# WangYuTum/odometry

Hardware: AMD Instinct MI355X
Metric: tracked frames/sec (1241x376, 4-level pyramid) (higher is better)
Workload: dtype f32

## Files before the change

### odometry_amd/csrc/kernels.hip.h

```cpp
#pragma once
#include <hip/hip_runtime.h>
#include "odo_math.h"

#ifndef ODO_PHASE_STAMPS
#define ODO_PHASE_STAMPS 0
#endif
#if ODO_PHASE_STAMPS
#define ODO_DBG(a) ((a).dbg)
#else
#define ODO_DBG(a) ((unsigned long long*)nullptr)
#endif

#ifndef ODO_KERNEL
#define ODO_KERNEL __global__
#define ODO_KERNEL_T __global__
#endif
#ifdef ODO_LM_CHAIN_TU
#define ODO_DEVICE_VAR static __device__
#else
#define ODO_DEVICE_VAR __device__
#endif

namespace odo {

// ... 915 lines not shown
  int n_levels;
  const LmState* st_in;
  LmState* st_out;
  const double* part_in;
  double* part_out;
  float lambda0, precision;
  int robust;
  float huber_delta;
  LmTraceRow* trace;
  float* cost_stat;
  int* host_prog;
  int seq;
  int first_of_solve;
  float init[16];
  unsigned long long* dbg;
  float* out;
  int* done_flag;
  int token;
  LmState* st2[2];
  double* part2[2];
  int min_level;
  int fine_lo;
  unsigned long long* xbuf;
  unsigned fine_dispatch;
  unsigned fine_epoch;
  unsigned fine_wait;
  int fine_home;
  float* chain_pose;
  int* chain_guard;
  int chain_in_token;
  int chain_out;
  float kf_rule[7];
  int stop_level;
  LmState* final_state;
  unsigned long long* span;
  unsigned long long* arm;
};
struct StepLaunch {
  const LmState* st_in; LmState* st_out;
  const double* part_in; double* part_out;
  int seq, first_of_solve;
  unsigned long long* span;
};
static_assert(offsetof(StepArgs, lv) == 0, "lm_copy_levels reads the level table at offset 0 of the StepArgs");
__device__ __forceinline__ const unsigned* lm_kernarg_words() { return (const unsigned*)__builtin_amdgcn_kernarg_segment_ptr(); }
__device__ __forceinline__ void lm_copy_levels(StepLevel* lv_sh, const unsigned* __restrict__ src) {
  constexpr int kWords = (int)(sizeof(StepLevel) * ODO_MAX_LEVELS_K / sizeof(unsigned));
  for (int i = (int)threadIdx.x; i < kWords; i += (int)blockDim.x) ((unsigned*)lv_sh)[i] = src[i];
}
__device__ __forceinline__ bool lm_span_block() {
  return threadIdx.x == 0 && (gridDim.y == 1 || ((blockIdx.x ^ blockIdx.y) & 7u) == 0u);
}
__device__ __forceinline__ void lm_span_begin(unsigned long long* span) {
  if (span && lm_span_block()) atomicMin(span, (unsigned long long)wall_clock64());
}
__device__ __forceinline__ void lm_span_end(unsigned long long* span) {
  if (span && lm_span_block()) atomicMax(span + 1, (unsigned long long)wall_clock64());
}

constexpr int kFoldChunk = 20;

__device__ __forceinline__ void lm_state_machine(bool pending, const StepLevel* lv, int n_levels, float lambda0,
                                                 float precision, LmState& s_sh, double* acc_sh, LmTraceRow* __restrict__ trace,
                                                 float* __restrict__ cost_stat, bool publisher,
                                                 unsigned long long* smdbg = nullptr, int stop_level = 0) {
  const int t = threadIdx.x;
  if (t < 64) {
    unsigned long long c0 = smdbg ? __builtin_readcyclecounter() : 0, c1 = c0, c2 = c0, c3 = c0;
    LmState s = s_sh;
    const int iter0 = s.iter, lvl0 = s.level;
    const float err_last0 = s.err_last;
    bool need_step = false;
    if (pending) need_step = lm_decide(&s, acc_sh, precision);
    if (smdbg) { c1 = __builtin_readcyclecounter(); c2 = c1; c3 = c1; }
    if (need_step) {
      float d[6];
      solve_damped_wave_regs(acc_sh, s.lambda, d);
#pragma unroll
      for (int i = 0; i < 6; i++) s.delta[i] = d[i];
      if (smdbg) { asm volatile("" ::"v"(d[0]), "v"(d[5])); c2 = __builtin_readcyclecounter(); }
#ifdef ODO_NO_LANE_SINCOS
      lm_apply_step(&s, s.max_iters);
#else
      lm_apply_step_wave(&s, s.max_iters);
#endif
      if (smdbg) { asm volatile("" ::"v"(s.T[0]), "v"(s.T[14])); c3 = __builtin_readcyclecounter(); }
    }
    if (smdbg && t == 0) { smdbg[0] += c1 - c0; smdbg[1] += c2 - c1; smdbg[2] += c3 - c2; smdbg[3] += 1; }
    if (pending) {
      if (publisher && t == 0 && trace) {
        const int ev = s.n_evals - 1;
        if (ev < kTraceCap) {
          LmTraceRow& r = trace[ev];
          r.level = lvl0;
          r.iter = iter0;
          r.n_res = (int)acc_sh[28];
          r.err = s.err_now;
          r.accepted = (s.status == 0 && !(s.err_now > err_last0)) ? 1 : 0;
          r.stop = (s.stop_reason == 3 || s.active) ? 0 : s.stop_reason;
          r.lambda_after = s.lambda;
#pragma unroll
          for (int i = 0; i < 6; i++) r.delta[i] = (s.active || s.stop_reason == 3) ? s.delta[i] : 0.0f;
        }
        int evals_this_level = 0;
#pragma unroll
        for (int i = 0; i < 8; i++) evals_this_level += (i == (lvl0 & 7)) ? s.iters_level[i] : 0;
        if (iter0 == 0 && evals_this_level == 1) cost_stat[lvl0 * 2 + 0] = s.err_now;
        cost_stat[lvl0 * 2 + 1] = s.err_now;
      }
      s.pending = 0;
    }
    if (lv) {
      while (!s.active && s.status == 0 && !s.finished) {
        const int next = (s.level < 0) ? n_levels - 1 : s.level - 1;
        if (next < stop_level) { s.finished = 1; break; }
        s.stop_reason = 0;
        lm_begin_level(&s, next, lambda0, lv[next].max_iters);
      }
      if (s.status != 0) s.finished = 1;
    }
    if (t == 0) s_sh = s;
  }
  __syncthreads();
}

struct LmHot {
  Se3 cur, inc;
  float Tc[12];
  float lambda, err_last;
  int level, iter, max_iters, active, status, finished, n_evals, stop_reason;
};
__device__ __forceinline__ void lm_hot_load(LmHot& h, const LmState& s) {
  h.cur = s.cur; h.inc = s.inc;
  float M[16];
  se3_to_colmajor(s.cur, M);
#pragma unroll
  for (int c = 0; c < 4; c++)
#pragma unroll
    for (int r = 0; r < 3; r++) h.Tc[c * 3 + r] = M[c * 4 + r];
  h.lambda = s.lambda; h.err_last = s.err_last;
  h.level = s.level; h.iter = s.iter; h.max_iters = s.max_iters; h.active = s.active; h.status = s.status; h.finished = s.finished;
  h.n_evals = s.n_evals; h.stop_reason = s.stop_reason;
}
__device__ __forceinline__ void lm_hot_store(const LmHot& h, LmState& s) {
  s.cur = h.cur; s.inc = h.inc; s.last = h.cur;
  s.lambda = h.lambda; s.err_last = h.err_last;
  s.level = h.level; s.iter = h.iter; s.max_iters = h.max_iters; s.active = h.active; s.status = h.status; s.finished = h.finished;
  s.n_evals = h.n_evals; s.stop_reason = h.stop_reason;
  s.pending = 0;
}
__device__ __forceinline__ void lm_state_machine_hot(LmHot& h, const StepLevel* lv, int n_levels, float lambda0, float precision,
                                                     LmState& s_sh, const double* acc_sh, LmTraceRow* __restrict__ trace,
                                                     float* __restrict__ cost_stat, bool publisher,
                                                     unsigned long long* smdbg = nullptr, int stop_level = 0) {
  const int t = threadIdx.x;
  if (t < 64) {
    unsigned long long c0 = smdbg ? __builtin_readcyclecounter() : 0, c1 = c0, c2 = c0, c3 = c0;
    const int iter0 = h.iter, lvl0 = h.level;
    const float err_last0 = h.err_last;
    float Tprev[12];
#pragma unroll
    for (int c = 0; c < 4; c++)
#pragma unroll
      for (int r = 0; r < 3; r++) Tprev[c * 3 + r] = s_sh.T[c * 4 + r];
    h.n_evals++;
    if (t == 0) s_sh.iters_level[lvl0 & 7] += 1;
    bool need_step = false;
    float err_now = 0.0f;
    bool have_err = false;
    if (!(acc_sh[28] > 0.0)) {
      h.status = -1;
      h.active = 0;
    } else {
      err_now = (float)(acc_sh[27] / acc_sh[28]);
      have_err = true;
      if (err_now > h.err_last) {
        h.lambda = h.lambda * 5.0f;
        if (h.lambda > 1e+5f) { h.active = 0; h.stop_reason = 2; }
        else need_step = true;
      } else {
        h.cur = h.inc;
#pragma unroll
        for (int i = 0; i < 12; i++) h.Tc[i] = Tprev[i];
        const float err_diff = err_now / h.err_last;
        if (err_diff > precision) { h.active = 0; h.stop_reason = 1; }
        else {
          h.err_last = err_now;
          h.lambda = fmaxf(h.lambda / 5.0f, 1e-5f);
          need_step = true;
        }
      }
    }
    if (smdbg) { c1 = __builtin_readcyclecounter(); c2 = c1; c3 = c1; }
    float d[6] = {0.0f, 0.0f, 0.0f, 0.0f, 0.0f, 0.0f};
    bool new_T = false;
    float Tn[16];
#pragma unroll
    for (int i = 0; i < 16; i++) Tn[i] = 0.0f;
    if (need_step) {
      solve_damped_wave_regs(acc_sh, h.lambda, d);
      if (smdbg) { asm volatile("" ::"v"(d[0]), "v"(d[5])); c2 = __builtin_readcyclecounter(); }
      Se3 dd;
      se3_exp_wave(d, &dd);
      const float C[16] = {h.Tc[0], h.Tc[1], h.Tc[2], 0.0f, h.Tc[3], h.Tc[4], h.Tc[5], 0.0f,
                           h.Tc[6], h.Tc[7], h.Tc[8], 0.0f, h.Tc[9], h.Tc[10], h.Tc[11], 1.0f};
      se3_left_update_mat(dd, C, &h.inc);
      se3_to_colmajor(h.inc, Tn);
      new_T = true;
      h.iter++;
      if (!(h.max_iters > h.iter)) { h.active = 0; h.stop_reason = 3; }
      if (smdbg) { asm volatile("" ::"v"(Tn[0]), "v"(Tn[14])); c3 = __builtin_readcyclecounter(); }
    }
    if (smdbg && t == 0) { smdbg[0] += c1 - c0; smdbg[1] += c2 - c1; smdbg[2] += c3 - c2; smdbg[3] += 1; }
    if (t == 0) {
      if (have_err) s_sh.err_now = err_now;
      if (need_step) {
#pragma unroll
        for (int i = 0; i < 6; i++) s_sh.delta[i] = d[i];
      }
    }
    if (publisher && t == 0 && trace) {
      const int ev = h.n_evals - 1;
      const float e = s_sh.err_now;
      if (ev < kTraceCap) {
        LmTraceRow& r = trace[ev];
        r.level = lvl0;
        r.iter = iter0;
        r.n_res = (int)acc_sh[28];
        r.err = e;
        r.accepted = (h.status == 0 && !(e > err_last0)) ? 1 : 0;
        r.stop = (h.stop_reason == 3 || h.active) ? 0 : h.stop_reason;
        r.lambda_after = h.lambda;
#pragma unroll
        for (int i = 0; i < 6; i++) r.delta[i] = (h.active || h.stop_reason == 3) ? d[i] : 0.0f;
      }
      const int evals_this_level = s_sh.iters_level[lvl0 & 7];
      if (iter0 == 0 && evals_this_level == 1) cost_stat[lvl0 * 2 + 0] = e;
      cost_stat[lvl0 * 2 + 1] = e;
    }
    if (lv) {
      while (!h.active && h.status == 0 && !h.finished) {
        const int next = (h.level < 0) ? n_levels - 1 : h.level - 1;
        if (next < stop_level) { h.finished = 1; break; }
        h.stop_reason = 0;
        h.level = next;
        h.iter = 0;
        h.err_last = 1e+10f;
        h.lambda = lambda0;
        h.inc = h.cur;
        h.max_iters = lv[next].max_iters;
        h.active = (h.status == 0 && h.max_iters > 0) ? 1 : 0;
#pragma unroll
        for (int c = 0; c < 4; c++) {
#pragma unroll
          for (int r = 0; r < 3; r++) Tn[c * 4 + r] = h.Tc[c * 3 + r];
          Tn[c * 4 + 3] = (c == 3) ? 1.0f : 0.0f;
        }
        new_T = true;
      }
      if (h.status != 0) h.finished = 1;
    }
    if (t == 0) {
      if (new_T) {
#pragma unroll
        for (int i = 0; i < 16; i++) s_sh.T[i] = Tn[i];
      }
      s_sh.level = h.level; s_sh.active = h.active; s_sh.status = h.status; s_sh.finished = h.finished;
    }
  }
  __syncthreads();
}

constexpr int kUpdThreads = 1024;
#define ODO_STAMP(i) do { if (STAMP && threadIdx.x == 0) stamps[i] = __builtin_readcyclecounter(); } while (0)
template <bool STAMP>
__device__ __forceinline__ void lm_update_body(LmState* __restrict__ st, const double* __restrict__ partials,
                                               int nblk, int expect_level, float precision, int max_iters,
                                               LmTraceRow* __restrict__ trace, float* __restrict__ cost_stat,
                                               int* __restrict__ host_prog, int seq,
                                               unsigned long long* __restrict__ stamps) {
  ODO_STAMP(0);
  if (!(st->active != 0 && st->level == expect_level)) {
    if (host_prog && threadIdx.x == 0) __hip_atomic_store(host_prog, seq, __ATOMIC_RELAXED, __HIP_MEMORY_SCOPE_SYSTEM);
    return;
  }
  __shared__ double sh[32][32];
  __shared__ double acc_sh[32];
  __shared__ LmState s_sh;
  const int t = threadIdx.x;
  const int q = t & 31, seg = t >> 5;
  double v = 0.0;
  if (q < ODO_NACC) {
    double v0 = 0.0, v1 = 0.0, v2 = 0.0, v3 = 0.0;
    int b = seg;
    for (; b + 96 < nblk; b += 128) {
      v0 += partials[(size_t)b * ODO_NACC + q];
      v1 += partials[(size_t)(b + 32) * ODO_NACC + q];
      v2 += partials[(size_t)(b + 64) * ODO_NACC + q];
      v3 += partials[(size_t)(b + 96) * ODO_NACC + q];
    }
    for (; b < nblk; b += 32) v0 += partials[(size_t)b * ODO_NACC + q];
    v = (v0 + v1) + (v2 + v3);
  }
  ODO_STAMP(1);
  sh[seg][q] = v;
  if (t < (int)(sizeof(LmState) / sizeof(int))) ((int*)&s_sh)[t] = ((const int*)st)[t];
  __syncthreads();
  if (t < ODO_NACC) {
    double a = 0.0;
// ... 465 lines not shown
}
static __global__ void __launch_bounds__(kCoarseBlock) lm_coarse_armed_kernel(StepArgs a, int min_level) {
  const StepLaunch q = {a.st_in, a.st_out, a.part_in, a.part_out, a.seq, a.first_of_solve, a.span};
  lm_coarse_body<false, true>(a, q, min_level, lm_kernarg_words());
}
static __global__ void __launch_bounds__(kCoarseBlock) lm_coarse_full_kernel(StepArgs a, int min_level) {
  const StepLaunch q = {a.st_in, a.st_out, a.part_in, a.part_out, a.seq, a.first_of_solve, a.span};
  lm_coarse_body<true>(a, q, min_level, lm_kernarg_words());
}
#endif
template <bool kFull>
__device__ __forceinline__ void lm_coarse_batch_entry(const StepArgs* __restrict__ table, int seq, int first_of_solve, unsigned long long* span) {
  const StepArgs& a = table[blockIdx.y];
  const StepLaunch q = {a.st2[seq & 1], a.st2[(seq + 1) & 1], a.part2[seq & 1], a.part2[(seq + 1) & 1], seq, first_of_solve, span};
  lm_coarse_body<kFull>(a, q, a.min_level, (const unsigned*)&table[blockIdx.y]);
}
ODO_KERNEL void __launch_bounds__(kCoarseBlock) lm_coarse_kernel_batch(const StepArgs* __restrict__ table, int seq, int first_of_solve,
                                                                       unsigned long long* span) {
  lm_coarse_batch_entry<false>(table, seq, first_of_solve, span);
}
ODO_KERNEL void __launch_bounds__(kCoarseBlock) lm_coarse_full_kernel_batch(const StepArgs* __restrict__ table, int seq, int first_of_solve,
                                                                            unsigned long long* span) {
  lm_coarse_batch_entry<true>(table, seq, first_of_solve, span);
}

constexpr int kFineGran = 2 * ODO_NACC;
constexpr int kFineRowsMax = 160;
constexpr int kFineChunk = 8;
constexpr unsigned kFineWaitTicks = 400000u;
struct FineDeadline {
  unsigned long long t0, c0;
  unsigned limit;
  static __device__ __forceinline__ FineDeadline begin(unsigned limit_ticks) {
    return FineDeadline{(unsigned long long)wall_clock64(), (unsigned long long)__builtin_readcyclecounter(), limit_ticks};
  }
  __device__ __forceinline__ bool expired(int spin) const {
    if ((spin & 31) != 31) return false;
    const unsigned long long dt = (unsigned long long)wall_clock64() - t0;
    if (dt <= (unsigned long long)limit) return false;
    if (dt > 4ull * (unsigned long long)limit) return true;
    return (unsigned long long)__builtin_readcyclecounter() - c0 > 24ull * (unsigned long long)limit;
  }
};
constexpr int kTsThreads = 512, kTsPerThread = 32, kTsMaxWg = 128;
constexpr int kTsXbufWords = 2 * kTsMaxWg * 4;
ODO_KERNEL void __launch_bounds__(kTsThreads) lm_tdist_scale_multi_kernel(const float* __restrict__ res, int n,
                                                                          const LmState* __restrict__ st, int expect_level,
                                                                          float* __restrict__ scale_sqr_out,
                                                                          unsigned long long* __restrict__ xbuf, unsigned epoch,
                                                                          unsigned wait_ticks, int* __restrict__ gave_up, int fault) {
  if (!(st->active != 0 && st->level == expect_level)) return;
  const int G = gridDim.x, g = blockIdx.x, t = threadIdx.x, lane = t & 63, wv = t >> 6;
  const size_t stride = (size_t)G * kTsThreads;
  float e2[kTsPerThread];
  int cnt = 0;
#pragma unroll
  for (int k = 0; k < kTsPerThread; k++) {
    const size_t i = (size_t)g * kTsThreads + t + (size_t)k * stride;
    const float r = (i < (size_t)n) ? res[i] : __builtin_nanf("");
    const bool ok = (r == r);
    e2[k] = ok ? r * r : -1.0f;
    cnt += ok ? 1 : 0;
  }
  __shared__ double wsum[kTsThreads / 64];
  __shared__ double wcnt[kTsThreads / 64];
  __shared__ float sh_sigma;
  __shared__ int sh_done, sh_bail;
  const unsigned wait_limit = wait_ticks ? wait_ticks : 400000u;
  float cur = 5.0f;
  double n_valid = 0.0;
  for (int pass = 0; pass < kTdistMaxPasses; pass++) {
    const float sigma_sqr = cur * cur;
    double s = 0.0;
#pragma unroll
    for (int k = 0; k < kTsPerThread; k++)
      if (e2[k] >= 0.0f) s += (double)tdist_term(e2[k], sigma_sqr);
    const double ws = wave_sum64(s);
    if (pass == 0) {
      const double wc = wave_sum64((double)cnt);
      if (lane == 0) wcnt[wv] = wc;
    }
    if (lane == 0) wsum[wv] = ws;
    __syncthreads();
    if (t < 64) {
      double P = 0.0, C = 0.0;
#pragma unroll
      for (int w = 0; w < kTsThreads / 64; w++) { P += wsum[w]; if (pass == 0) C += wcnt[w]; }
      const unsigned tag = (epoch << 10) | (unsigned)(pass + 1);
      unsigned long long* mine = xbuf + ((size_t)(pass & 1) * kTsMaxWg + g) * 4;
      if (lane == 0 && !(fault && g == 1)) {
        const unsigned long long bits = (unsigned long long)__double_as_longlong(P);
        __hip_atomic_store(mine + 0, ((bits >> 32) << 32) | tag, __ATOMIC_RELAXED, __HIP_MEMORY_SCOPE_AGENT);
        __hip_atomic_store(mine + 1, ((bits & 0xffffffffull) << 32) | tag, __ATOMIC_RELAXED, __HIP_MEMORY_SCOPE_AGENT);
        __hip_atomic_store(mine + 2, ((unsigned long long)(unsigned)(int)C << 32) | tag, __ATOMIC_RELAXED, __HIP_MEMORY_SCOPE_AGENT);
      }
      double a = 0.0, c = 0.0;
      bool all = true;
      const FineDeadline dl = FineDeadline::begin(wait_limit);
      for (int gg = lane; gg < G; gg += 64) {
        const unsigned long long* theirs = xbuf + ((size_t)(pass & 1) * kTsMaxWg + gg) * 4;
        unsigned long long w0 = 0, w1 = 0, w2 = 0;
        bool got = false;
        for (int spin = 0; !got; spin++) {
          w0 = __hip_atomic_load(theirs + 0, __ATOMIC_RELAXED, __HIP_MEMORY_SCOPE_AGENT);
          w1 = __hip_atomic_load(theirs + 1, __ATOMIC_RELAXED, __HIP_MEMORY_SCOPE_AGENT);
          w2 = __hip_atomic_load(theirs + 2, __ATOMIC_RELAXED, __HIP_MEMORY_SCOPE_AGENT);
          got = ((unsigned)w0 == tag) && ((unsigned)w1 == tag) && ((unsigned)w2 == tag);
          if (!got && dl.expired(spin)) break;
        }
        all = all && got;
        a += __longlong_as_double((long long)(((w0 >> 32) << 32) | (w1 >> 32)));
        c += (double)(int)(unsigned)(w2 >> 32);
      }
      const bool everyone = __all(all);
      const double total = wave_sum64(a);
      if (pass == 0) n_valid = wave_sum64(c);
      const float nxt = (n_valid > 0.0) ? tdist_next_sigma(total, (int)n_valid) : cur;
      const bool done = !(n_valid > 0.0) || tdist_converged(nxt, cur);
      if (lane == 0) { sh_sigma = nxt; sh_done = done ? 1 : 0; sh_bail = everyone ? 0 : 1; }
    }
    __syncthreads();
    if (sh_bail) {
      if (t == 0) __hip_atomic_store(gave_up, 1, __ATOMIC_RELAXED, __HIP_MEMORY_SCOPE_AGENT);
      return;
    }
    cur = sh_sigma;
    if (sh_done) break;
  }
  if (g == 0 && t == 0) *scale_sqr_out = cur * cur;
}

constexpr int kFineThreads = 2 * kLmBlock;
constexpr int kFineKMax = 32;
constexpr int kScaleChunks = 4 * 2 * kFineKMax;
constexpr int kScaleWords = 2 * kScaleChunks * 2 + kScaleChunks;
constexpr int kFineScaleOff = 2 * kFineRowsMax * kFineGran + kFineKMax;
static_assert(kFineScaleOff % 2 == 0, "scale granule pairs must be 16-byte aligned");
constexpr int kFineXbufWords = kFineScaleOff + kScaleWords;
constexpr int kTdistMaxEvals = 1023;
typedef unsigned FineG2 __attribute__((ext_vector_type(4)));
typedef __attribute__((address_space(1))) FineG2 FineG2Global;
__device__ __forceinline__ void fine_publish(unsigned long long* __restrict__ buf, int vb, int q, double acc, unsigned tag, bool local) {
  const unsigned long long bits = (unsigned long long)__double_as_longlong(acc);
  unsigned long long* g = buf + (size_t)vb * kFineGran + 2 * q;
  const unsigned long long g0 = ((bits >> 32) << 32) | tag, g1 = (bits << 32) | tag;
  if (local) {
    g[0] = g0;
    g[1] = g1;
  } else {
    __hip_atomic_store(g, g0, __ATOMIC_RELAXED, __HIP_MEMORY_SCOPE_AGENT);
    __hip_atomic_store(g + 1, g1, __ATOMIC_RELAXED, __HIP_MEMORY_SCOPE_AGENT);
  }
}
__device__ __forceinline__ int fine_xcc_id() {
  int v;
  asm volatile("s_getreg_b32 %0, hwreg(HW_REG_XCC_ID)" : "=s"(v));
  return v & 0xf;
}
__device__ __forceinline__ bool fine_on_home(int home) {
  return home >= 0 ? fine_xcc_id() == home : (blockIdx.x & 7u) == 0u;
}
ODO_KERNEL void xcc_probe_kernel(int* __restrict__ out) {
  if (threadIdx.x == 0) out[blockIdx.x] = fine_xcc_id();
}
struct XccIds { int id[8]; };
__device__ __forceinline__ float fine_tdist_sigma(unsigned long long* __restrict__ sbuf, int chunk, int nchunk, unsigned tag_ev,
                                                          float e2, bool valid, bool local, unsigned wait_limit, int* bail,
                                                          double (*td_ws)[8], int* td_cnt) {
  const int lane = threadIdx.x & 63, wv = threadIdx.x >> 6;
  const int vb = chunk >> 2, nvb = nchunk >> 2;
  unsigned long long* cnts = sbuf + 2 * kScaleChunks * 2;
  const int my_cnt = __popcll(__ballot(valid));
  float sigma = 5.0f;
  int n_total = 0;
  for (int pass = 0; pass < kTdistMaxPasses; pass++) {
    const unsigned tag = tag_ev | (unsigned)(pass + 1);
    const double ws = wave_sum64(valid ? (double)tdist_term(e2, sigma * sigma) : 0.0);
    if (lane == 0) { td_ws[pass & 1][wv] = ws; if (pass == 0) td_cnt[wv] = my_cnt; }
    __syncthreads();
    unsigned long long* sums = sbuf + (size_t)(pass & 1) * kScaleChunks * 2;
    if ((wv & 3) == 0 && lane == 0) {
      const double G = ((td_ws[pass & 1][wv] + td_ws[pass & 1][wv + 1]) + td_ws[pass & 1][wv + 2]) + td_ws[pass & 1][wv + 3];
      const int C = td_cnt[wv] + td_cnt[wv + 1] + td_cnt[wv + 2] + td_cnt[wv + 3];
      const unsigned long long bits = (unsigned long long)__double_as_longlong(G);
      const unsigned long long g0 = ((bits >> 32) << 32) | tag, g1 = (bits << 32) | tag;
      const unsigned long long gc = ((unsigned long long)(unsigned)C << 32) | tag;
      if (local) {
        sums[2 * vb] = g0; sums[2 * vb + 1] = g1;
        if (pass == 0) cnts[vb] = gc;
      } else {
        __hip_atomic_store(sums + 2 * vb, g0, __ATOMIC_RELAXED, __HIP_MEMORY_SCOPE_AGENT);
        __hip_atomic_store(sums + 2 * vb + 1, g1, __ATOMIC_RELAXED, __HIP_MEMORY_SCOPE_AGENT);
        if (pass == 0) __hip_atomic_store(cnts + vb, gc, __ATOMIC_RELAXED, __HIP_MEMORY_SCOPE_AGENT);
      }
    }
    FineG2 g = {0, 0, 0, 0};
    unsigned long long gc = 0;
    bool all = false;
    FineDeadline dl = {0ull, 0ull, wait_limit};
    __builtin_amdgcn_s_setprio(0);
    for (int spin = 0; !all; spin++) {
      if (spin == 1) dl = FineDeadline::begin(wait_limit);
      if (spin > 0) { if (dl.expired(spin)) break; __builtin_amdgcn_s_sleep(1); }
      bool mine = true;
      if (lane < nvb) {
        g = *(const volatile FineG2Global*)(sums + 2 * lane);
        if (pass == 0) gc = __hip_atomic_load(cnts + lane, __ATOMIC_RELAXED, __HIP_MEMORY_SCOPE_AGENT);
        mine = (g.x == tag) && (g.z == tag) && (pass != 0 || (unsigned)gc == tag);
      }
      all = __all(mine);
    }
    __builtin_amdgcn_s_setprio(3);
    if (!all) { if (lane == 0) *bail = 1; break; }
    double part = 0.0, cnt = 0.0;
    if (lane < nvb) {
      part = __longlong_as_double((long long)(((unsigned long long)g.y << 32) | (unsigned long long)g.w));
      if (pass == 0) cnt = (double)(unsigned)(gc >> 32);
    }
    const double total = wave_sum64(part);
    if (pass == 0) n_total = (int)wave_sum64(cnt);
    const float nxt = (n_total > 0) ? tdist_next_sigma(total, n_total) : sigma;
    const bool done = (n_total == 0) || tdist_converged(nxt, sigma);
    sigma = nxt;
    if (done) break;
  }
  return sigma;
}
template <bool kTdist, bool kTrace>
__device__ __forceinline__ void lm_fine_body(const StepArgs& a, const StepLaunch& q, int K, int w, unsigned long long* __restrict__ xbuf,
                                             int fault, int lo_level, const unsigned* __restrict__ lv_src) {
#if ODO_PHASE_STAMPS
  const unsigned long long w_entry = (unsigned long long)wall_clock64();
#endif
  __builtin_amdgcn_s_setprio(3);
  const int t = threadIdx.x, tl = t & (kLmBlock - 1), half = t >> 8;
  const bool publisher = (w == 0);
  if (publisher && t == 0 && q.span) atomicMin(q.span, (unsigned long long)wall_clock64());
  __shared__ LmState s_sh;
  __shared__ double fold_sh[8 * 32];
  __shared__ double acc_sh[32];
  __shared__ StepLevel lv_sh[ODO_MAX_LEVELS_K];
  __shared__ float rows_sh2[2][kRowFloats * RowBuf<kLmBlock>::W];
  __shared__ int bail_sh, local_sh;
  __shared__ unsigned long long sm_sh[4];
  float* rows_sh = rows_sh2[half];
  const unsigned tag_base = a.fine_epoch << 8;
  unsigned long long* place = xbuf + 2 * kFineRowsMax * kFineGran;
  const unsigned wait_limit = a.fine_wait ? a.fine_wait : kFineWaitTicks;
  lm_copy_levels(lv_sh, lv_src);
  if (t == 0) {
    bail_sh = 0;
    local_sh = 0;
#pragma unroll
    for (int i = 0; i < 4; i++) sm_sh[i] = 0;
    __hip_atomic_store(place + w, ((unsigned long long)(unsigned)fine_xcc_id() << 32) | tag_base, __ATOMIC_RELAXED, __HIP_MEMORY_SCOPE_AGENT);
  }
  __syncthreads();
  lm_fused_prologue(q.st_in, q.part_in, lv_sh, a.n_levels, a.lambda0, a.precision, s_sh, fold_sh, acc_sh, (kTrace ? a.trace : (LmTraceRow*)nullptr), a.cost_stat,
                    publisher, q.first_of_solve ? a.init : nullptr, a.stop_level, a.chain_in_token ? a.chain_pose : nullptr);
  LmHot hot;
  lm_hot_load(hot, s_sh);
  if (t < 64) {
    bool same = true, got = false;
    if (t < K) {
      unsigned long long pw = 0;
      const FineDeadline dl = FineDeadline::begin(wait_limit);
      for (int spin = 0; !got; spin++) {
        pw = __hip_atomic_load(place + t, __ATOMIC_RELAXED, __HIP_MEMORY_SCOPE_AGENT);
        got = ((unsigned)pw == tag_base);
        if (!got && dl.expired(spin)) break;
      }
      same = got && ((int)(pw >> 32) == fine_xcc_id());
    } else {
      got = true;
    }
    const bool all_got = __all(got), all_same = __all(same);
    if (t == 0) { local_sh = (all_got && all_same) ? 1 : 0; if (!all_got) bail_sh = 1; }
  }
  __syncthreads();
  const bool local = local_sh != 0;
  constexpr int kS = 8;
  const int my_q = tl / kS, my_s = tl % kS;
  int rowA = 0, rowB = 0;
  if (my_q < ODO_NACC) rows_of_quantity(my_q, &rowA, &rowB);
  const int fq = t & 31, fseg = t >> 5;
  PointK pt;
  bool pt_ok = false;
  int pt_level = -1;
  unsigned long long c_eval = 0, c_xchg = 0, c_sm = 0, c_it = 0, c_last = ODO_DBG(a) ? __builtin_readcyclecounter() : 0;
#if ODO_PHASE_STAMPS
  unsigned long long c_first = 0, n_first = 0;
#endif
  const unsigned long long c_begin = c_last, w_begin = ODO_DBG(a) ? (unsigned long long)wall_clock64() : 0;
  auto lap = [&](unsigned long long& sum) {
    if (ODO_DBG(a)) { const unsigned long long now = __builtin_readcyclecounter(); sum += now - c_last; c_last = now; }
  };
  for (int ev = 0; ev < 4096; ev++) {
    const bool run = (s_sh.active != 0 && s_sh.status == 0 && !s_sh.finished && !bail_sh && s_sh.level >= lo_level);
    if (!run) break;
    c_it++;
    const StepLevel& L = lv_sh[s_sh.level];
    const float* I2u = lm_uniform_ptr(L.I2);
    const int nblk = L.nblk;
    const unsigned tag = tag_base + 1u + (unsigned)(ev % 255);
    unsigned long long* buf = xbuf + (size_t)(ev & 1) * kFineRowsMax * kFineGran;
    float T[16];
#pragma unroll
    for (int i = 0; i < 16; i++) T[i] = s_sh.T[i];
#if ODO_PHASE_STAMPS
    const bool first_of_level = (s_sh.level != pt_level);
#endif
    const bool resident = (nblk <= 2 * K) && (L.n <= nblk * kLmBlock);
    if (resident) {
      const int vb = w + half * K;
      if (s_sh.level != pt_level) {
        pt_level = s_sh.level;
        const int idx = vb * kLmBlock + tl;
        pt_ok = vb < nblk && idx < L.n;
        if (pt_ok) pt = load_point(L.pl, idx);
      }
      float r = 0.0f, wgt = 0.0f, J[6] = {0.0f, 0.0f, 0.0f, 0.0f, 0.0f, 0.0f};
      bool valid = false;
      if (pt_ok && point_residual_g<kTdist || kTrace>(pt, T, L.k, I2u, L.rows, L.cols, &r, J)) {
        wgt = robust_weight(r, (kTdist || kTrace) ? a.robust : (a.robust == 1 ? 1 : 0), a.huber_delta, 1.0f);
        valid = true;
      }
      if (kTdist && w < nblk) {
        __shared__ double td_ws_sh[2][8];
        __shared__ int td_cnt_sh[8];
        const float sg = fine_tdist_sigma(xbuf + kFineScaleOff, vb * 4 + (tl >> 6), 4 * nblk,
                                          ((a.fine_epoch & 0xfffu) << 20) | (((unsigned)ev & 0x3ffu) << 10), r * r, valid, local, wait_limit, &bail_sh,
                                          td_ws_sh, td_cnt_sh);
        if (valid) wgt = robust_weight(r, 2, a.huber_delta, sg * sg);
      }
      rows_store_z(rows_sh, RowBuf<kLmBlock>::W, tl, J, wgt, r, valid);
      __syncthreads();
      if (bail_sh) break;
      if (vb < nblk) {
        double accq = 0.0;
        if (my_q < ODO_NACC) accq = rows_accumulate<kLmBlock, kS>(rows_sh, rowA, rowB, my_s, accq);
        accq = rows_butterfly8(accq);
        if (my_q < ODO_NACC && my_s == 0 && !(fault && vb == 0)) fine_publish(buf, vb, my_q, accq, tag, local);
      }
    } else {
      const int rounds = (L.n + nblk * kLmBlock - 1) / (nblk * kLmBlock);
      for (int vb0 = w; vb0 < nblk; vb0 += 2 * K) {
        const int vb = vb0 + half * K;
        double accq = 0.0;
        for (int rd = 0; rd < rounds; rd++) {
          const int idx = (vb + rd * nblk) * kLmBlock + tl;
          float r = 0.0f, wgt = 0.0f, J[6] = {0.0f, 0.0f, 0.0f, 0.0f, 0.0f, 0.0f};
          bool valid = false;
          if (vb < nblk && idx < L.n) {
            const PointK p = load_point(L.pl, idx);
            if (point_residual_g<kTdist || kTrace>(p, T, L.k, I2u, L.rows, L.cols, &r, J)) {
              wgt = robust_weight(r, (kTdist || kTrace) ? a.robust : (a.robust == 1 ? 1 : 0), a.huber_delta, 1.0f);
              valid = true;
            }
          }
          __syncthreads();
          rows_store_z(rows_sh, RowBuf<kLmBlock>::W, tl, J, wgt, r, valid);
          __syncthreads();
          if (my_q < ODO_NACC) accq = rows_accumulate<kLmBlock, kS>(rows_sh, rowA, rowB, my_s, accq);
        }
        accq = rows_butterfly8(accq);
        if (vb < nblk && my_q < ODO_NACC && my_s == 0 && !(fault && vb == 0)) fine_publish(buf, vb, my_q, accq, tag, local);
      }
    }
#if ODO_PHASE_STAMPS
    { const unsigned long long before = c_eval; lap(c_eval); if (first_of_level) { c_first += c_eval - before; n_first++; } }
#else
    lap(c_eval);
#endif
    double v = 0.0;
    __builtin_amdgcn_s_setprio(0);
    if (fq < ODO_NACC && fseg < 8) {
      for (int b0 = fseg; b0 < nblk; b0 += 8 * kFineChunk) {
        FineG2 g2[kFineChunk];
        bool all = false;
        FineDeadline dl = {0ull, 0ull, wait_limit};
        for (int spin = 0; !all; spin++) {
          if (spin == 1) dl = FineDeadline::begin(wait_limit);
          if (spin > 0) { if (dl.expired(spin)) break; __builtin_amdgcn_s_sleep(1); }
          all = true;
#pragma unroll
          for (int u = 0; u < kFineChunk; u++) {
            const int b = b0 + 8 * u;
            if (b < nblk) g2[u] = *(const volatile FineG2Global*)(buf + (size_t)b * kFineGran + 2 * fq);
          }
#pragma unroll
          for (int u = 0; u < kFineChunk; u++) {
            const int b = b0 + 8 * u;
            if (b < nblk) all = all && (g2[u].x == tag) && (g2[u].z == tag);
          }
        }
        if (!all) bail_sh = 1;
#pragma unroll
        for (int u = 0; u < kFineChunk; u++) {
          const int b = b0 + 8 * u;
          if (b < nblk) v += __longlong_as_double((long long)(((unsigned long long)g2[u].y << 32) | (unsigned long long)g2[u].w));
        }
      }
    }
    __builtin_amdgcn_s_setprio(3);
    if (fseg < 8) fold_sh[fseg * 32 + fq] = v;
    __syncthreads();
    if (t < ODO_NACC) {
      double acc = 0.0;
#pragma unroll
      for (int g = 0; g < 8; g++) acc += fold_sh[g * 32 + t];
      acc_sh[t] = acc;
    }
    lap(c_xchg);
    if (bail_sh) break;
    lm_state_machine_hot(hot, lv_sh, a.n_levels, a.lambda0, a.precision, s_sh, acc_sh, (kTrace ? a.trace : (LmTraceRow*)nullptr), a.cost_stat, publisher,
                         (ODO_DBG(a) && publisher) ? sm_sh : nullptr, a.stop_level);
    lap(c_sm);
  }
#if ODO_PHASE_STAMPS
  const unsigned long long w_loop_end = (unsigned long long)wall_clock64();
#endif
  if (t == 0) lm_hot_store(hot, s_sh);
  if (bail_sh && t == 0) { s_sh.status = -2; s_sh.active = 0; s_sh.finished = 1; }
  __syncthreads();
  if (publisher) {
    lm_fused_publish(s_sh, q.st_out, a.host_prog, q.seq, a.token, a.cost_stat, a.out, a.done_flag, a.final_state, chain_out_of(a));
#if ODO_PHASE_STAMPS
    const unsigned long long w_published = (unsigned long long)wall_clock64();
#endif
    if (ODO_DBG(a) && t == 0) { ODO_DBG(a)[128] += c_eval; ODO_DBG(a)[129] += c_xchg; ODO_DBG(a)[130] += c_sm; ODO_DBG(a)[131] += c_it; ODO_DBG(a)[132] += 1; ODO_DBG(a)[133] += local ? 1 : 0;
      ODO_DBG(a)[134] += __builtin_readcyclecounter() - c_begin; ODO_DBG(a)[135] += (unsigned long long)wall_clock64() - w_begin;
#pragma unroll
      for (int i = 0; i < 4; i++) ODO_DBG(a)[136 + i] += sm_sh[i]; }
    if (t == 0 && q.span) atomicMax(q.span + 1, (unsigned long long)wall_clock64());
#if ODO_PHASE_STAMPS
    if (ODO_DBG(a) && t == 0) {
      const unsigned long long now = w_published;
      g_lm_diag[2] = w_loop_end;
      g_lm_diag[19] += c_first; g_lm_diag[20] += n_first;
      g_lm_diag[9] += w_begin - w_entry; g_lm_diag[10] += w_loop_end - w_begin; g_lm_diag[11] += now - w_loop_end;
      if (g_lm_diag[0] && w_entry > g_lm_diag[0] && w_entry - g_lm_diag[0] < 100000ull) { g_lm_diag[12] += w_entry - g_lm_diag[0]; g_lm_diag[15] += 1; }
      g_lm_diag[1] = now; g_lm_diag[13] += 1;
    }
#endif
  }
}
ODO_DEVICE_VAR unsigned g_lm_fine_dispatch[2];
__device__ __forceinline__ bool lm_fine_mid_dispatch() {
  return __hip_atomic_load(&g_lm_fine_dispatch[0], __ATOMIC_RELAXED, __HIP_MEMORY_SCOPE_AGENT) !=
         __hip_atomic_load(&g_lm_fine_dispatch[1], __ATOMIC_RELAXED, __HIP_MEMORY_SCOPE_AGENT);
}
template <bool kTdist, bool kTrace>
__device__ __forceinline__ void lm_fine_entry(const StepArgs& a, int K, unsigned long long* __restrict__ xbuf, int fault, int lo_level,
                                              unsigned* dispatch_words) {
  if (threadIdx.x == 0) {
    if (blockIdx.x == 0) __hip_atomic_store(&dispatch_words[0], a.fine_dispatch, __ATOMIC_RELAXED, __HIP_MEMORY_SCOPE_AGENT);
    if (blockIdx.x == gridDim.x - 1) __hip_atomic_store(&dispatch_words[1], a.fine_dispatch, __ATOMIC_RELAXED, __HIP_MEMORY_SCOPE_AGENT);
  }
  if (!fine_on_home(a.fine_home) || lm_chain_skip(a)) return;
  const StepLaunch q = {a.st_in, a.st_out, a.part_in, a.part_out, a.seq, a.first_of_solve, a.span};
  lm_fine_body<kTdist, kTrace>(a, q, K, (int)(blockIdx.x >> 3), xbuf, fault, lo_level, lm_kernarg_words());
}
#ifdef ODO_LM_CHAIN_TU
static __global__ void __launch_bounds__(kFineThreads) lm_fine_kernel(StepArgs a, int K, unsigned long long* __restrict__ xbuf, int fault,
                                                               int lo_level, unsigned* dispatch_words) {
  lm_fine_entry<false, false>(a, K, xbuf, fault, lo_level, dispatch_words);
}
static __global__ void __launch_bounds__(kFineThreads) lm_fine_trace_kernel(StepArgs a, int K, unsigned long long* __restrict__ xbuf, int fault,
                                                                     int lo_level, unsigned* dispatch_words) {
  lm_fine_entry<false, true>(a, K, xbuf, fault, lo_level, dispatch_words);
}
static __global__ void __launch_bounds__(kFineThreads) lm_fine_tdist_kernel(StepArgs a, int K, unsigned long long* __restrict__ xbuf, int fault,
                                                                     int lo_level, unsigned* dispatch_words) {
  lm_fine_entry<true, true>(a, K, xbuf, fault, lo_level, dispatch_words);
}
#endif
template <bool kTrace>
__device__ __forceinline__ void lm_fine_batch_entry(const StepArgs* __restrict__ table, int n, int K, int seq, int first_of_solve,
                                                    unsigned long long* span, int fault, const XccIds& xcc, unsigned* dispatch_words) {
  int r = (int)(blockIdx.x & 7u);
  if (xcc.id[0] >= 0) {
    const int mine = fine_xcc_id();
#pragma unroll
    for (int c = 0; c < 8; c++) if (xcc.id[c] == mine) r = c;
  }
  if (threadIdx.x == 0 && n > 0) {
    if (blockIdx.x == 0) __hip_atomic_store(&dispatch_words[0], table[0].fine_dispatch, __ATOMIC_RELAXED, __HIP_MEMORY_SCOPE_AGENT);
    if (blockIdx.x == gridDim.x - 1) __hip_atomic_store(&dispatch_words[1], table[0].fine_dispatch, __ATOMIC_RELAXED, __HIP_MEMORY_SCOPE_AGENT);
  }
  const int wa = (int)(blockIdx.x >> 3);
  const int i = (wa / K) * 8 + r, w = wa % K;
  if (i >= n) return;
  const StepArgs& a = table[i];
  const StepLaunch q = {a.st2[seq & 1], a.st2[(seq + 1) & 1], a.part2[seq & 1], a.part2[(seq + 1) & 1], seq, first_of_solve,
                        (i == 0) ? span : nullptr};
  if (a.fine_lo >= a.min_level) {
    if (w == 0) lm_fine_body<false, kTrace>(a, q, 1, 0, a.xbuf, 0, ODO_MAX_LEVELS_K + 1, (const unsigned*)&table[i]);
    return;
  }
  lm_fine_body<false, kTrace>(a, q, K, w, a.xbuf, fault, a.fine_lo, (const unsigned*)&table[i]);
}
ODO_KERNEL void __launch_bounds__(kFineThreads) lm_fine_kernel_batch(const StepArgs* __restrict__ table, int n, int K, int seq,
                                                                     int first_of_solve, unsigned long long* span, int fault, XccIds xcc,
                                                                     unsigned* dispatch_words) {
  lm_fine_batch_entry<false>(table, n, K, seq, first_of_solve, span, fault, xcc, dispatch_words);
}
ODO_KERNEL void __launch_bounds__(kFineThreads) lm_fine_trace_kernel_batch(const StepArgs* __restrict__ table, int n, int K, int seq,
                                                                           int first_of_solve, unsigned long long* span, int fault, XccIds xcc,
                                                                     unsigned* dispatch_words) {
  lm_fine_batch_entry<true>(table, n, K, seq, first_of_solve, span, fault, xcc, dispatch_words);
}

struct FinalizeArgs {
  const LmState* st_in;
  const double* part_in;
  float precision;
  LmTraceRow* trace;
  float* cost_stat;
  LmState* st_out;
  float* out;
  int* done_flag;
  int token;
  int first_of_solve;
  float init[16];
};
ODO_KERNEL void __launch_bounds__(kLmBlock) lm_fused_finalize_kernel(FinalizeArgs a) {
  __shared__ LmState s_sh;
  __shared__ double fold_sh[8 * 32];
  __shared__ double acc_sh[32];
  lm_fused_prologue(a.st_in, a.part_in, nullptr, 0, 0.0f, a.precision, s_sh, fold_sh, acc_sh, a.trace,
                    a.cost_stat, true, a.first_of_solve ? a.init : nullptr);
  if (threadIdx.x < (int)(sizeof(LmState) / sizeof(int))) ((int*)a.st_out)[threadIdx.x] = ((const int*)&s_sh)[threadIdx.x];
  if (threadIdx.x == 0) lm_write_result(s_sh, a.cost_stat, a.out, a.done_flag, a.token);
}

ODO_KERNEL void solve_damped_wave_test_kernel(const double* __restrict__ acc_in, float lambda, float* __restrict__ out) {
  __shared__ double acc_sh[32];
  __shared__ float delta_sh[6];
  if (threadIdx.x < ODO_NACC) acc_sh[threadIdx.x] = acc_in[threadIdx.x];
  __syncthreads();
  solve_damped_wave(acc_sh, lambda, delta_sh);
  __syncthreads();
  if (threadIdx.x < 6) out[threadIdx.x] = delta_sh[threadIdx.x];
}

ODO_KERNEL void lm_begin_solve_kernel(LmState* __restrict__ st, const float* __restrict__ init, float* __restrict__ cost_stat) {
  if (threadIdx.x == 0) {
    LmState s;
    float m[16];
    for (int i = 0; i < 16; i++) m[i] = init[i];
    lm_begin_solve(&s, m);
    s.level = -1; s.iter = 0; s.lambda = 0.0f; s.err_last = 1e+10f;
    for (int i = 0; i < 16; i++) s.T[i] = m[i];
    *st = s;
    for (int i = 0; i < 16; i++) cost_stat[i] = 0.0f;
  }
}

ODO_KERNEL void lm_begin_level_kernel(LmState* __restrict__ st, int level, float lambda0, int max_iters) {
  if (threadIdx.x == 0) {
    LmState s = *st;
    s.stop_reason = 0;
    lm_begin_level(&s, level, lambda0, max_iters);
    *st = s;
  }
}

__device__ __forceinline__ void lm_finalize_body(const LmState* __restrict__ st, float* __restrict__ out);
ODO_KERNEL void lm_finalize_kernel(const LmState* __restrict__ st, float* __restrict__ out) { lm_finalize_body(st, out); }
ODO_KERNEL void lm_finalize_batch_kernel(const UpdItem* __restrict__ items) { lm_finalize_body(items[blockIdx.x].st, items[blockIdx.x].out); }
ODO_KERNEL void lm_begin_solve_batch_kernel(const UpdItem* __restrict__ items) {
  if (threadIdx.x == 0) {
    const UpdItem& q = items[blockIdx.x];
    LmState s;
    float m[16];
    for (int i = 0; i < 16; i++) m[i] = q.init[i];
    lm_begin_solve(&s, m);
    s.level = -1; s.iter = 0; s.lambda = 0.0f; s.err_last = 1e+10f;
    for (int i = 0; i < 16; i++) s.T[i] = m[i];
    *q.st = s;
    for (int i = 0; i < 16; i++) q.cost_stat[i] = 0.0f;
  }
}
ODO_KERNEL void lm_begin_level_batch_kernel(const UpdItem* __restrict__ items) {
  if (threadIdx.x == 0) {
    const UpdItem& q = items[blockIdx.x];
    LmState s = *q.st;
    s.stop_reason = 0;
    lm_begin_level(&s, q.expect_level, q.lambda0, q.max_iters);
    *q.st = s;
  }
}
__device__ __forceinline__ void lm_finalize_body(const LmState* __restrict__ st, float* __restrict__ out) {
  if (threadIdx.x == 0) {
    float m[16];
    if (st->status == 0) {
      se3_to_colmajor(st->cur, m);
    } else {
      for (int i = 0; i < 16; i++) m[i] = 0.0f;
      m[0] = 1.0f; m[5] = 1.0f; m[10] = 1.0f;
    }
    for (int i = 0; i < 16; i++) out[i] = m[i];
    out[16] = (float)st->status;
    out[17] = (float)st->n_evals;
    for (int i = 0; i < 8; i++) out[18 + i] = (float)st->iters_level[i];
  }
}

constexpr int kSelCap = 80;
constexpr int kSelBlocks = 512;
#ifndef ODO_SEL_THREADS
#define ODO_SEL_THREADS 512
#endif
constexpr int kSelThreads = ODO_SEL_THREADS;
constexpr int kSelMaxElems = 4096;

__device__ __forceinline__ void depth_select_kernel_body(const float* __restrict__ L, int rows, int cols, int bnd,
                                                                    float grad_th, uint8_t* __restrict__ val,
                                                                    uint32_t* __restrict__ pts, int* __restrict__ cnt) {
  __shared__ float mag[kSelMaxElems];
  __shared__ int wave_tot[kSelThreads / kWave];
  __shared__ int base_sh;
  const int t = threadIdx.x;
  const int bw = (cols - bnd * 2) / 32, bh = (rows - bnd * 2) / 16;
  const int bsz = bw * bh;
  const int b = blockIdx.x;
  if (bsz <= 0 || bsz > kSelMaxElems) {
    if (t == 0) cnt[b] = 0;
    return;
  }
  const int sy = bnd + (b / 32) * bh, sx = bnd + (b % 32) * bw;
  constexpr int kPer = kSelMaxElems / kSelThreads;
  unsigned keys[kPer];
#pragma unroll
  for (int u = 0; u < kPer; u++) {
    const int e = t + u * kSelThreads;
    keys[u] = 0xffffffffu;
    if (e < bsz) {
      const int y = sy + e / bw, x = sx + e % bw;
      const float gx = 0.5f * (L[(size_t)y * cols + x + 1] - L[(size_t)y * cols + x - 1]);
      const float gy = 0.5f * (L[(size_t)(y + 1) * cols + x] - L[(size_t)(y - 1) * cols + x]);
      const float m = sqrtf(gx * gx + gy * gy);
      mag[e] = m;
      keys[u] = __float_as_uint(m);
    }
  }
  __syncthreads();
  __shared__ int hist[256];
  __shared__ int sel_sh[2];
  unsigned prefix = 0u, pmask = 0u;
  int kth = bsz / 2;
  {
    const int lane = t & 63;
// ... 668 lines not shown
```

Measured before the change: 4088.

## Add single-wave fast path for small fine-level reductions and skip placement handshake

When the number of publishing blocks is small (at most eight rows) and resident, one wavefront polls the tagged partial sums, folds them with a permlane32 swap and writes acc_sh directly. This avoids the eight-segment gather, the fold_sh write and a block-wide __syncthreads per LM iteration. It also skips the XCC placement publish/spin handshake and its barrier when placement is already known (home XCC set or xcc ids provided), and gates the state machine on whether sums arrived. The risk is correctness if a bail in the solo path is not propagated the same way, and extra code complexity.

After: 4280, median of 6. +4.7%, better.

```diff
diff --git a/odometry_amd/csrc/kernels.hip.h b/odometry_amd/csrc/kernels.hip.h
--- a/odometry_amd/csrc/kernels.hip.h
+++ b/odometry_amd/csrc/kernels.hip.h
@@ -1091,9 +1091,9 @@
 __device__ __forceinline__ void lm_state_machine_hot(LmHot& h, const StepLevel* lv, int n_levels, float lambda0, float precision,
                                                      LmState& s_sh, const double* acc_sh, LmTraceRow* __restrict__ trace,
                                                      float* __restrict__ cost_stat, bool publisher,
-                                                     unsigned long long* smdbg = nullptr, int stop_level = 0) {
+                                                     unsigned long long* smdbg = nullptr, int stop_level = 0, bool have_sums = true) {
   const int t = threadIdx.x;
-  if (t < 64) {
+  if (t < 64 && have_sums) {
     unsigned long long c0 = smdbg ? __builtin_readcyclecounter() : 0, c1 = c0, c2 = c0, c3 = c0;
     const int iter0 = h.iter, lvl0 = h.level;
     const float err_last0 = h.err_last;
@@ -1865,6 +1865,16 @@
     __hip_atomic_store(g + 1, g1, __ATOMIC_RELAXED, __HIP_MEMORY_SCOPE_AGENT);
   }
 }
+constexpr int kFineSoloRows = 8;
+constexpr int kFineSoloU = kFineSoloRows / 8;
+static_assert(kFineSoloRows % 8 == 0 && kFineSoloRows <= 8 * kFineChunk, "whole segments, one chunk of the four-wave gather");
+__device__ __forceinline__ double fine_upper_half(double x) {
+  const unsigned long long b = (unsigned long long)__double_as_longlong(x);
+  const unsigned lo = (unsigned)b, hi = (unsigned)(b >> 32);
+  const auto rl = __builtin_amdgcn_permlane32_swap(lo, lo, false, false);
+  const auto rh = __builtin_amdgcn_permlane32_swap(hi, hi, false, false);
+  return __longlong_as_double((long long)(((unsigned long long)rh[1] << 32) | (unsigned long long)rl[1]));
+}
 __device__ __forceinline__ int fine_xcc_id() {
   int v;
   asm volatile("s_getreg_b32 %0, hwreg(HW_REG_XCC_ID)" : "=s"(v));
@@ -1941,7 +1951,7 @@
 }
 template <bool kTdist, bool kTrace>
 __device__ __forceinline__ void lm_fine_body(const StepArgs& a, const StepLaunch& q, int K, int w, unsigned long long* __restrict__ xbuf,
-                                             int fault, int lo_level, const unsigned* __restrict__ lv_src) {
+                                             int fault, int lo_level, const unsigned* __restrict__ lv_src, bool placed) {
 #if ODO_PHASE_STAMPS
   const unsigned long long w_entry = (unsigned long long)wall_clock64();
 #endif
@@ -1966,14 +1976,14 @@
     local_sh = 0;
 #pragma unroll
     for (int i = 0; i < 4; i++) sm_sh[i] = 0;
-    __hip_atomic_store(place + w, ((unsigned long long)(unsigned)fine_xcc_id() << 32) | tag_base, __ATOMIC_RELAXED, __HIP_MEMORY_SCOPE_AGENT);
+    if (!placed) __hip_atomic_store(place + w, ((unsigned long long)(unsigned)fine_xcc_id() << 32) | tag_base, __ATOMIC_RELAXED, __HIP_MEMORY_SCOPE_AGENT);
   }
   __syncthreads();
   lm_fused_prologue(q.st_in, q.part_in, lv_sh, a.n_levels, a.lambda0, a.precision, s_sh, fold_sh, acc_sh, (kTrace ? a.trace : (LmTraceRow*)nullptr), a.cost_stat,
                     publisher, q.first_of_solve ? a.init : nullptr, a.stop_level, a.chain_in_token ? a.chain_pose : nullptr);
   LmHot hot;
   lm_hot_load(hot, s_sh);
-  if (t < 64) {
+  if (!placed && t < 64) {
     bool same = true, got = false;
     if (t < K) {
       unsigned long long pw = 0;
@@ -1990,8 +2000,8 @@
     const bool all_got = __all(got), all_same = __all(same);
     if (t == 0) { local_sh = (all_got && all_same) ? 1 : 0; if (!all_got) bail_sh = 1; }
   }
-  __syncthreads();
-  const bool local = local_sh != 0;
+  if (!placed) __syncthreads();
+  const bool local = placed || local_sh != 0;
   constexpr int kS = 8;
   const int my_q = tl / kS, my_s = tl % kS;
   int rowA = 0, rowB = 0;
@@ -2085,49 +2095,108 @@
 #else
     lap(c_eval);
 #endif
-    double v = 0.0;
-    __builtin_amdgcn_s_setprio(0);
-    if (fq < ODO_NACC && fseg < 8) {
-      for (int b0 = fseg; b0 < nblk; b0 += 8 * kFineChunk) {
-        FineG2 g2[kFineChunk];
+    bool have_sums = true;
+    if (resident && nblk <= kFineSoloRows) {
+      if (t < 64) {
+        const int sq = t & 31, sg0 = 4 * (t >> 5), nrel = nblk - sg0;
+        const unsigned long long* row0 = buf + (size_t)sg0 * kFineGran + 2 * sq;
+        unsigned long long gh[4][kFineSoloU] = {}, gl[4][kFineSoloU] = {};
         bool all = false;
         FineDeadline dl = {0ull, 0ull, wait_limit};
+        __builtin_amdgcn_s_setprio(0);
         for (int spin = 0; !all; spin++) {
           if (spin == 1) dl = FineDeadline::begin(wait_limit);
           if (spin > 0) { if (dl.expired(spin)) break; __builtin_amdgcn_s_sleep(1); }
-          all = true;
+          bool mine = true;
+          if (sq < ODO_NACC) {
+#pragma unroll
+            for (int j = 0; j < 4; j++)
+#pragma unroll
+              for (int u = 0; u < kFineSoloU; u++)
+                if (j + 8 * u < nrel) {
+                  gh[j][u] = __hip_atomic_load(row0 + (j + 8 * u) * kFineGran, __ATOMIC_RELAXED, __HIP_MEMORY_SCOPE_AGENT);
+                  gl[j][u] = __hip_atomic_load(row0 + (j + 8 * u) * kFineGran + 1, __ATOMIC_RELAXED, __HIP_MEMORY_SCOPE_AGENT);
+                }
+#pragma unroll
+            for (int j = 0; j < 4; j++)
+#pragma unroll
+              for (int u = 0; u < kFineSoloU; u++)
+                if (j + 8 * u < nrel) mine = mine && ((unsigned)gh[j][u] == tag) && ((unsigned)gl[j][u] == tag);
+          }
+          all = __all(mine);
+        }
+        __builtin_amdgcn_s_setprio(3);
+        double vs[4] = {0.0, 0.0, 0.0, 0.0}, up[4];
+        if (sq < ODO_NACC) {
+#pragma unroll
+          for (int j = 0; j < 4; j++)
+#pragma unroll
+            for (int u = 0; u < kFineSoloU; u++)
+              if (j + 8 * u < nrel) vs[j] += __longlong_as_double((long long)(((gh[j][u] >> 32) << 32) | (gl[j][u] >> 32)));
+        }
+#pragma unroll
+        for (int j = 0; j < 4; j++) up[j] = fine_upper_half(vs[j]);
+        if (t < ODO_NACC) {
+          double acc = 0.0;
+#pragma unroll
+          for (int j = 0; j < 4; j++) acc += vs[j];
+#pragma unroll
+          for (int j = 0; j < 4; j++) acc += up[j];
+          acc_sh[t] = acc;
+        }
+        have_sums = all;
+        if (!all && t == 0) bail_sh = 1;
+      }
+      lap(c_xchg);
+    } else {
+      double v = 0.0;
+      __builtin_amdgcn_s_setprio(0);
+      if (fq < ODO_NACC && fseg < 8) {
+        for (int b0 = fseg; b0 < nblk; b0 += 8 * kFineChunk) {
+          FineG2 g2[kFineChunk] = {};
+          bool all = false;
+          FineDeadline dl = {0ull, 0ull, wait_limit};
+          for (int spin = 0; !all; spin++) {
+            if (spin == 1) dl = FineDeadline::begin(wait_limit);
+            if (spin > 0) { if (dl.expired(spin)) break; __builtin_amdgcn_s_sleep(1); }
+            all = true;
+#pragma unroll
+            for (int u = 0; u < kFineChunk; u++) {
+              const int b = b0 + 8 * u;
+              if (b < nblk) {
+                const unsigned long long h = __hip_atomic_load(buf + (size_t)b * kFineGran + 2 * fq, __ATOMIC_RELAXED, __HIP_MEMORY_SCOPE_AGENT);
+                const unsigned long long l = __hip_atomic_load(buf + (size_t)b * kFineGran + 2 * fq + 1, __ATOMIC_RELAXED, __HIP_MEMORY_SCOPE_AGENT);
+                g2[u].x = (unsigned)h; g2[u].y = (unsigned)(h >> 32); g2[u].z = (unsigned)l; g2[u].w = (unsigned)(l >> 32);
+              }
+            }
+#pragma unroll
+            for (int u = 0; u < kFineChunk; u++) {
+              const int b = b0 + 8 * u;
+              if (b < nblk) all = all && (g2[u].x == tag) && (g2[u].z == tag);
+            }
+          }
+          if (!all) bail_sh = 1;
 #pragma unroll
           for (int u = 0; u < kFineChunk; u++) {
             const int b = b0 + 8 * u;
-            if (b < nblk) g2[u] = *(const volatile FineG2Global*)(buf + (size_t)b * kFineGran + 2 * fq);
-          }
-#pragma unroll
-          for (int u = 0; u < kFineChunk; u++) {
-            const int b = b0 + 8 * u;
-            if (b < nblk) all = all && (g2[u].x == tag) && (g2[u].z == tag);
+            if (b < nblk) v += __longlong_as_double((long long)(((unsigned long long)g2[u].y << 32) | (unsigned long long)g2[u].w));
           }
         }
-        if (!all) bail_sh = 1;
-#pragma unroll
-        for (int u = 0; u < kFineChunk; u++) {
-          const int b = b0 + 8 * u;
-          if (b < nblk) v += __longlong_as_double((long long)(((unsigned long long)g2[u].y << 32) | (unsigned long long)g2[u].w));
-        }
-      }
-    }
-    __builtin_amdgcn_s_setprio(3);
-    if (fseg < 8) fold_sh[fseg * 32 + fq] = v;
-    __syncthreads();
-    if (t < ODO_NACC) {
-      double acc = 0.0;
-#pragma unroll
-      for (int g = 0; g < 8; g++) acc += fold_sh[g * 32 + t];
-      acc_sh[t] = acc;
-    }
-    lap(c_xchg);
-    if (bail_sh) break;
+      }
+      __builtin_amdgcn_s_setprio(3);
+      if (fseg < 8) fold_sh[fseg * 32 + fq] = v;
+      __syncthreads();
+      if (t < ODO_NACC) {
+        double acc = 0.0;
+#pragma unroll
+        for (int g = 0; g < 8; g++) acc += fold_sh[g * 32 + t];
+        acc_sh[t] = acc;
+      }
+      lap(c_xchg);
+      if (bail_sh) break;
+    }
     lm_state_machine_hot(hot, lv_sh, a.n_levels, a.lambda0, a.precision, s_sh, acc_sh, (kTrace ? a.trace : (LmTraceRow*)nullptr), a.cost_stat, publisher,
-                         (ODO_DBG(a) && publisher) ? sm_sh : nullptr, a.stop_level);
+                         (ODO_DBG(a) && publisher) ? sm_sh : nullptr, a.stop_level, have_sums);
     lap(c_sm);
   }
 #if ODO_PHASE_STAMPS
@@ -2172,7 +2241,7 @@
   }
   if (!fine_on_home(a.fine_home) || lm_chain_skip(a)) return;
   const StepLaunch q = {a.st_in, a.st_out, a.part_in, a.part_out, a.seq, a.first_of_solve, a.span};
-  lm_fine_body<kTdist, kTrace>(a, q, K, (int)(blockIdx.x >> 3), xbuf, fault, lo_level, lm_kernarg_words());
+  lm_fine_body<kTdist, kTrace>(a, q, K, (int)(blockIdx.x >> 3), xbuf, fault, lo_level, lm_kernarg_words(), a.fine_home >= 0);
 }
 #ifdef ODO_LM_CHAIN_TU
 static __global__ void __launch_bounds__(kFineThreads) lm_fine_kernel(StepArgs a, int K, unsigned long long* __restrict__ xbuf, int fault,
@@ -2208,10 +2277,10 @@
   const StepLaunch q = {a.st2[seq & 1], a.st2[(seq + 1) & 1], a.part2[seq & 1], a.part2[(seq + 1) & 1], seq, first_of_solve,
                         (i == 0) ? span : nullptr};
   if (a.fine_lo >= a.min_level) {
-    if (w == 0) lm_fine_body<false, kTrace>(a, q, 1, 0, a.xbuf, 0, ODO_MAX_LEVELS_K + 1, (const unsigned*)&table[i]);
+    if (w == 0) lm_fine_body<false, kTrace>(a, q, 1, 0, a.xbuf, 0, ODO_MAX_LEVELS_K + 1, (const unsigned*)&table[i], true);
     return;
   }
-  lm_fine_body<false, kTrace>(a, q, K, w, a.xbuf, fault, a.fine_lo, (const unsigned*)&table[i]);
+  lm_fine_body<false, kTrace>(a, q, K, w, a.xbuf, fault, a.fine_lo, (const unsigned*)&table[i], xcc.id[0] >= 0);
 }
 ODO_KERNEL void __launch_bounds__(kFineThreads) lm_fine_kernel_batch(const StepArgs* __restrict__ table, int n, int K, int seq,
                                                                      int first_of_solve, unsigned long long* span, int fault, XccIds xcc,
```
